# AUTOMATIC1111/stable-diffusion-webui

Hardware: AMD Instinct MI355X
Metric: images/sec SD1.5 512x512 20-step Euler-a, batch 8 per GPU (higher is better)
Workload: dtype f16

## Files before the change

### include/sdmi.h

```cpp
#ifndef SDMI_H
#define SDMI_H

#include <stdint.h>

#ifdef __cplusplus
extern "C" {
#endif

#define SDMI_VERSION 100

enum { SDMI_F16 = 0, SDMI_F32 = 1 };

typedef struct sdmi_engine sdmi_engine;

int sdmi_version(void);
const char* sdmi_last_error(void);
int sdmi_device_ok(void);


int64_t sdmi_attention_workspace_bytes(int B, int H, int M, int D);
int sdmi_attention(const void* q, const void* k, const void* v, void* out,
                   int B, int H, int N, int M, int D,
                   int ldq, int ldk, int ldv, int ldo, float scale,
                   void* workspace, int64_t workspace_bytes, void* stream);
// ... 32 lines not shown
    int32_t force_generic;
    int32_t reserved;
    void* splitk_workspace;
    int64_t splitk_workspace_bytes;
} sdmi_conv_desc;

enum {
    SDMI_EP_OUT_F32  = 1,
    SDMI_EP_GEGLU    = 2,
    SDMI_EP_NCHW     = 4,
    SDMI_EP_BIAS_ROW = 8,
    SDMI_EP_WRAP = 128,
    SDMI_EP_TRANSPOSE = 64
};
int sdmi_conv_gemm(const sdmi_conv_desc* d, void* stream);
int64_t sdmi_conv_splitk_workspace_bytes(int M, int N, int K, int batch);

int sdmi_pack_conv_weight(const void* w_oihw, int dtype, void* out_f16, int O, int I, int kh, int kw,
                          int O_pad, int I_pad, int geglu, void* stream);

int sdmi_groupnorm(const void* x0, const void* x1, int c0, int c1, const void* gamma_f32, const void* beta_f32,
                   void* out_f16, int B, int HW, int groups, float eps, int silu,
                   void* workspace_f32, int64_t workspace_bytes, void* stream);
int64_t sdmi_groupnorm_workspace_bytes(int B, int HW, int groups);

int sdmi_layernorm(const void* x, const void* gamma_f32, const void* beta_f32, void* out_f16,
                   int64_t rows, int C, float eps, void* stream);

int64_t sdmi_rowchain_ff_pack_bytes(int C, int hidden);
int sdmi_rowchain_ff_pack(const void* w1_f16, const void* b1_f32_or_null, const void* w2_f16, void* packs, int C, int hidden,
                          void* stream);
int sdmi_rowchain_ff(const void* x_f16, void* out_f16, const void* ln_gamma_f32, const void* ln_beta_f32, const void* packs,
                     const void* b2_f32_or_null, int64_t rows, int C, int hidden, float eps, void* stream);


int sdmi_philox_randn(void* out_f32, int64_t n, uint64_t seed, uint32_t offset, void* stream);

int sdmi_slerp(void* out_f32, const void* low_f32, const void* high_f32, float val, int C, int H, int W, void* scratch_f32,
               void* stream);


int sdmi_cfg_prepare_input(const void* x_f32, const void* c_in_f32, void* x_in, int out_dtype,
                           int B, int reps, int64_t chw, void* stream);

int sdmi_cfg_prepare_concat(const void* x_f32, const void* c_in_f32, const void* c_concat_f32, void* x_in, int out_dtype,
                            int B, int reps, int C, int Cc, int64_t hw, uint32_t zero_reps, void* stream);

int sdmi_cfg_combine(const void* x_f32, const void* eps_f32, const void* c_out_f32, float cond_scale, int mode,
                     const void* mask_f32, const void* nmask_f32, const void* init_latent_f32,
                     void* denoised_f32, int B, int64_t chw, void* stream);

int sdmi_cfg_combine_affine(const void* x_f32, const void* out_f32, const void* c_out_f32, const void* c_skip_f32,
                            float cond_scale, const void* mask_f32, const void* nmask_f32, const void* init_latent_f32,
                            void* denoised_f32, int B, int64_t chw, void* stream);

int sdmi_euler_step(void* x_f32, const void* denoised_f32, const void* noise_f32_or_null,
                    float sigma, float sigma_down, float sigma_up, float s_noise, int64_t n, void* stream);

int sdmi_dpmpp2m_step(void* x_f32, const void* denoised_f32, const void* old_denoised_f32_or_null,
                      float ratio, float em1, float c1, float c2, int64_t n, void* stream);

int sdmi_ddim_step(void* x_f32, const void* e_t_f32, const void* noise_f32_or_null, void* pred_x0_f32_or_null,
                   float a_t, float a_prev, float sigma_t, float sqrt_one_minus_at, int64_t n, void* stream);

int sdmi_axpby(void* y_f32, const void* x_f32, float a, const void* z_f32_or_null, float b, int64_t n, void* stream);

// ... 218 lines not shown
```

### stable-diffusion-webui_amd/_lib.py

```python
from __future__ import annotations

import ctypes as C
import os
import re

_HERE = os.path.dirname(os.path.abspath(__file__))
LIB_PATH = os.environ.get("SDMI_LIB") or os.path.join(_HERE, "lib", "libsdmi.so")
HEADER_PATH = os.path.join(os.path.dirname(_HERE), "include", "sdmi.h")

F16, F32 = 0, 1
EP_OUT_F32, EP_GEGLU, EP_NCHW, EP_BIAS_ROW = 1, 2, 4, 8
EP_TRANSPOSE = 64
EP_WRAP = 128
RRDB_EP_NONE, RRDB_EP_LRELU, RRDB_EP_RES1, RRDB_EP_RES2 = 0, 1, 2, 3
RRDB_ST_F16, RRDB_ST_F32_NCHW, RRDB_ST_U8_HWC = 0, 1, 2
COMPACT_EP_NONE, COMPACT_EP_PRELU, COMPACT_EP_TAIL = 0, 1, 2


class SdmiError(RuntimeError):
    pass


class ConvDesc(C.Structure):
    _fields_ = [
# ... 66 lines not shown
def declared_symbols() -> list:
    src = open(HEADER_PATH).read()
    src = re.sub(r"/\*.*?\*/", "", src, flags=re.S)
    return sorted(set(re.findall(r"\b(sdmi_[a-z0-9_]+)\s*\(", src)))


if not os.path.exists(LIB_PATH):
    raise ImportError(
        f"{LIB_PATH} is missing: build it with `python -c 'import __graft_entry__ as g; g.build()'` "
        "(hipcc --offload-arch=gfx950). There is no CPU fallback for the MI355X engine.")

lib = C.CDLL(LIB_PATH)

_vp, _i, _i64, _f, _u32 = C.c_void_p, C.c_int, C.c_int64, C.c_float, C.c_uint32
_SIGS = {
    "sdmi_version": (C.c_int, []),
    "sdmi_last_error": (C.c_char_p, []),
    "sdmi_device_ok": (C.c_int, []),
    "sdmi_attention_workspace_bytes": (_i64, [_i, _i, _i, _i]),
    "sdmi_attention": (_i, [_vp, _vp, _vp, _vp, _i, _i, _i, _i, _i, _i, _i, _i, _i, _f, _vp, _i64, _vp]),
    "sdmi_attention_wide_workspace_bytes": (_i64, [_i, _i, _i, _i]),
    "sdmi_attention_wide": (_i, [_vp, _vp, _vp, _vp, _i, _i, _i, _i, _i, _i, _i, _i, _f, _vp, _i64, _vp]),
    "sdmi_attention_vt": (_i, [_vp, _vp, _vp, _vp, _i, _i, _i, _i, _i, _i, _i, _i, _i, _f, _i, _vp]),
    "sdmi_conv_gemm": (_i, [C.POINTER(ConvDesc), _vp]),
    "sdmi_conv_splitk_workspace_bytes": (_i64, [_i, _i, _i, _i]),
    "sdmi_bench_conv_gemm": (_i, [C.POINTER(ConvDesc), _i, C.POINTER(C.c_float), _vp]),
    "sdmi_pack_conv_weight": (_i, [_vp, _i, _vp, _i, _i, _i, _i, _i, _i, _i, _vp]),
    "sdmi_groupnorm": (_i, [_vp, _vp, _i, _i, _vp, _vp, _vp, _i, _i, _i, _f, _i, _vp, _i64, _vp]),
    "sdmi_groupnorm_workspace_bytes": (_i64, [_i, _i, _i]),
    "sdmi_layernorm": (_i, [_vp, _vp, _vp, _vp, _i64, _i, _f, _vp]),
    "sdmi_rowchain_ff_pack_bytes": (_i64, [_i, _i]),
    "sdmi_rowchain_ff_pack": (_i, [_vp, _vp, _vp, _vp, _i, _i, _vp]),
    "sdmi_rowchain_ff": (_i, [_vp, _vp, _vp, _vp, _vp, _vp, _i64, _i, _i, _f, _vp]),
    "sdmi_philox_randn": (_i, [_vp, _i64, C.c_uint64, C.c_uint32, _vp]),
    "sdmi_slerp": (_i, [_vp, _vp, _vp, _f, _i, _i, _i, _vp, _vp]),
    "sdmi_cfg_prepare_input": (_i, [_vp, _vp, _vp, _i, _i, _i, _i64, _vp]),
    "sdmi_cfg_prepare_concat": (_i, [_vp, _vp, _vp, _vp, _i, _i, _i, _i, _i, _i64, _u32, _vp]),
    "sdmi_cfg_combine": (_i, [_vp, _vp, _vp, _f, _i, _vp, _vp, _vp, _vp, _i, _i64, _vp]),
    "sdmi_cfg_combine_affine": (_i, [_vp, _vp, _vp, _vp, _f, _vp, _vp, _vp, _vp, _i, _i64, _vp]),
    "sdmi_euler_step": (_i, [_vp, _vp, _vp, _f, _f, _f, _f, _i64, _vp]),
    "sdmi_dpmpp2m_step": (_i, [_vp, _vp, _vp, _f, _f, _f, _f, _i64, _vp]),
    "sdmi_ddim_step": (_i, [_vp, _vp, _vp, _vp, _f, _f, _f, _f, _i64, _vp]),
    "sdmi_axpby": (_i, [_vp, _vp, _f, _vp, _f, _i64, _vp]),
    "sdmi_dpm_error_partials": (_i, [_vp, _vp, _vp, _f, _f, _vp, _i64, _vp]),
    "sdmi_lincomb": (_i, [_vp, C.POINTER(_vp), C.POINTER(_f), _i, _i64, _vp]),
    "sdmi_mask_blend": (_i, [_vp, _vp, _vp, _vp, _i64, _vp]),
    "sdmi_latent_resize": (_i, [_vp, _vp, _i, _i, _i, _i, _i, _i, _vp]),
    "sdmi_image_to_u8": (_i, [_vp, _vp, _i, _i, _i, _i, _vp]),
    "sdmi_engine_create": (_vp, [_i]),
    "sdmi_engine_destroy": (None, [_vp]),
    "sdmi_unet_configure": (_i, [_vp, C.POINTER(UNetConfigC)]),
    "sdmi_unet_load_tensor": (_i, [_vp, C.c_char_p, _vp, _i, _i, C.POINTER(C.c_int64), _i]),
    "sdmi_unet_finalize": (_i, [_vp]),
    "sdmi_clip_configure": (_i, [_vp, _i, C.POINTER(ClipConfigC)]),
    "sdmi_clip_load_tensor": (_i, [_vp, _i, C.c_char_p, _vp, _i, _i, C.POINTER(C.c_int64), _i]),
    "sdmi_clip_finalize": (_i, [_vp, _i]),
    "sdmi_clip_forward": (_i, [_vp, _i, _vp, _vp, _i, _i, _i, _i, _vp, _vp, _vp]),
    "sdmi_unet_update_weight": (_i, [_vp, C.c_char_p, _vp, _i, _i, C.POINTER(C.c_int64), _i]),
    "sdmi_unet_hypernet_clear": (_i, [_vp]),
    "sdmi_unet_hypernet_begin": (_i, [_vp, _f]),
    "sdmi_unet_hypernet_linear": (_i, [_vp, _i, _i, _vp, _vp, _i, _i, _i, _i]),
    "sdmi_unet_hypernet_act": (_i, [_vp, _i, _i, _i]),
    "sdmi_unet_hypernet_layernorm": (_i, [_vp, _i, _i, _vp, _vp, _i, _i, _i]),
    "sdmi_unet_update_vector": (_i, [_vp, C.c_char_p, _vp, _i, _i64, _i]),
    "sdmi_lora_merge": (_i, [_vp, _vp, _i, _vp, _i, _vp, _i, _i, _i, _i, _f, _vp]),
    "sdmi_weight_hadamard": (_i, [_vp, _vp, _vp, _vp, _f, _i64, _vp]),
# ... 83 lines not shown
```

### stable-diffusion-webui_amd/csrc/capi.cpp

```cpp
#include "engine.h"
#include "prof.h"
#include <cstring>

namespace sdmi {
extern int g_vae_attn_rows;
int unet_forward(sdmi_engine* e, const void* x, const void* t, const void* ctx, const void* y, void* out, int io_dtype,
                 int Bn, int h, int w, int L, hipStream_t s);
int vae_decode(sdmi_engine* e, const void* z, int io_dtype, float* out, int B, int h, int w, hipStream_t s);
int vae_encode(sdmi_engine* e, const void* x, int io_dtype, float* out, int B, int H, int W, hipStream_t s);
int engine_load_unet_tensor(sdmi_engine* e, const char* key, const void* data, int dtype, int ndim, const int64_t* shape, int on_device);
int engine_load_vae_tensor(sdmi_engine* e, const char* key, const void* data, int dtype, int ndim, const int64_t* shape, int on_device);
int engine_unet_finalize(sdmi_engine* e);
int engine_clip_configure(sdmi_engine* e, int slot, const sdmi_clip_config* cfg);
int engine_clip_load_tensor(sdmi_engine* e, int slot, const char* key, const void* data, int dtype, int ndim, const int64_t* shape, int on_device);
int engine_clip_finalize(sdmi_engine* e, int slot);
int engine_clip_forward(sdmi_engine* e, int slot, const int* tokens, const float* inputs_embeds, int B, int L, int skip,
                        int apply_final_ln, float* out, float* pooled, hipStream_t s);
int engine_unet_update_weight(sdmi_engine* e, const char* key, const void* data, int dtype, int ndim, const int64_t* shape, int on_device);
int engine_vae_finalize(sdmi_engine* e);
int engine_hypernet_clear(sdmi_engine* e);
int engine_hypernet_begin(sdmi_engine* e, float multiplier);
int engine_hypernet_linear(sdmi_engine* e, int dim, int which, const void* w, const void* b, int dtype, int out_f, int in_f, int on_device);
int engine_hypernet_act(sdmi_engine* e, int dim, int which, int act);
int engine_hypernet_layernorm(sdmi_engine* e, int dim, int which, const void* g, const void* b, int dtype, int n, int on_device);
// ... 202 lines not shown

int64_t sdmi_groupnorm_workspace_bytes(int B, int HW, int groups) { return groupnorm_ws_bytes(B, HW, groups); }

int sdmi_groupnorm(const void* x0, const void* x1, int c0, int c1, const void* gamma, const void* beta, void* out, int B, int HW,
                   int groups, float eps, int silu, void* ws, int64_t ws_bytes, void* stream) {
    API_GUARD_BEGIN
    SDMI_REQUIRE(ws && ws_bytes >= groupnorm_ws_bytes(B, HW, groups), "groupnorm workspace too small");
    return launch_groupnorm((const half_t*)x0, (const half_t*)x1, c0, x1 ? c1 : 0, (const float*)gamma, (const float*)beta,
                            (half_t*)out, B, HW, groups, eps, silu != 0, (float*)ws, (hipStream_t)stream);
    API_GUARD_END
}

int sdmi_layernorm(const void* x, const void* gamma, const void* beta, void* out, int64_t rows, int C, float eps, void* stream) {
    API_GUARD_BEGIN
    return launch_layernorm((const half_t*)x, (const float*)gamma, (const float*)beta, (half_t*)out, rows, C, eps, (hipStream_t)stream);
    API_GUARD_END
}

int64_t sdmi_rowchain_ff_pack_bytes(int C, int hidden) { return (int64_t)rowchain_ff_pack_bytes(C, hidden); }
int sdmi_rowchain_ff_pack(const void* w1, const void* b1, const void* w2, void* packs, int C, int hidden, void* stream) {
    API_GUARD_BEGIN
    SDMI_REQUIRE(w1 && w2 && packs, "null argument");
    return launch_rowchain_ff_pack((const half_t*)w1, (const float*)b1, (const half_t*)w2, packs, C, hidden, false, (hipStream_t)stream);
    API_GUARD_END
}
int sdmi_rowchain_ff(const void* x, void* out, const void* g, const void* b, const void* packs, const void* b2, int64_t rows, int C,
                     int hidden, float eps, void* stream) {
    API_GUARD_BEGIN
    SDMI_REQUIRE(x && out && g && b && packs, "null argument");
    return launch_rowchain_ff((const half_t*)x, (half_t*)out, (const float*)g, (const float*)b, packs, (const float*)b2, (long)rows, C,
                              hidden, eps, (hipStream_t)stream);
    API_GUARD_END
}


int sdmi_philox_randn(void* out, int64_t n, uint64_t seed, uint32_t offset, void* stream) {
    API_GUARD_BEGIN
    return launch_philox((float*)out, n, seed, offset, (hipStream_t)stream);
    API_GUARD_END
}

int sdmi_slerp(void* out, const void* low, const void* high, float val, int C, int H, int W, void* scratch, void* stream) {
    API_GUARD_BEGIN
    SDMI_REQUIRE(out && low && high && scratch && C > 0 && H > 0 && W > 0, "bad arguments");
    return launch_slerp((float*)out, (const float*)low, (const float*)high, val, C, H, W, (float*)scratch, (hipStream_t)stream);
    API_GUARD_END
}

int sdmi_cfg_prepare_input(const void* x, const void* c_in, void* x_in, int out_dtype, int B, int reps, int64_t chw, void* stream) {
    API_GUARD_BEGIN
    return launch_cfg_prepare((const float*)x, (const float*)c_in, x_in, out_dtype, B, reps, chw, (hipStream_t)stream);
    API_GUARD_END
}

int sdmi_cfg_prepare_concat(const void* x, const void* c_in, const void* c_concat, void* x_in, int out_dtype, int B, int reps,
                            int C, int Cc, int64_t hw, uint32_t zero_reps, void* stream) {
    API_GUARD_BEGIN
    SDMI_REQUIRE(x && c_concat && x_in, "null pointer");
    SDMI_REQUIRE(B > 0 && reps > 0 && reps <= 32 && C > 0 && Cc > 0 && hw > 0, "bad sizes");
    return launch_cfg_prepare_concat((const float*)x, (const float*)c_in, (const float*)c_concat, x_in, out_dtype, B, reps, C, Cc, hw,
                                     zero_reps, (hipStream_t)stream);
    API_GUARD_END
}

int sdmi_cfg_combine(const void* x, const void* eps, const void* c_out, float cond_scale, int mode, const void* mask,
                     const void* nmask, const void* init_latent, void* den, int B, int64_t chw, void* stream) {
// ... 532 lines not shown
```

### stable-diffusion-webui_amd/csrc/common.h

```cpp
#pragma once
#include <hip/hip_runtime.h>
#include <stdint.h>
#include <string>

typedef _Float16 half_t;
typedef _Float16 h8 __attribute__((ext_vector_type(8)));
typedef _Float16 h4 __attribute__((ext_vector_type(4)));
typedef _Float16 h2 __attribute__((ext_vector_type(2)));
typedef float f4 __attribute__((ext_vector_type(4)));
typedef float f16v __attribute__((ext_vector_type(16)));

namespace sdmi {

#ifndef SDMI_GELU_SIG
#define SDMI_GELU_SIG 1
#endif
__device__ __forceinline__ float geglu_gate(float val, float g) {
    const float gc = fminf(fmaxf(g, -10.0f), 10.0f);
    const float g2 = gc * gc;
    float p = fmaf(1.01426306e-3f, g2, -0.106775724f);
    p = fmaf(p, g2, -2.30112135f);
    const float e = __builtin_amdgcn_exp2f(p * gc);
    return (val * g) * __builtin_amdgcn_rcpf(1.0f + e);
}
// ... 116 lines not shown
extern int g_gemm_pipe_default;
extern int g_force_gemm_split;
extern int g_attn_kvt;
extern int g_attn_occ;
extern int g_attn_lds_pad;
extern int g_attn_fold_min_m;
extern int g_attn_tau;
extern unsigned long long g_attn_dbg;
extern int g_gemm_dbgflags;
extern unsigned long long g_gemm_dbg;

struct AttnP {
    const half_t* q;
    const half_t* k;
    const half_t* vt;
    half_t* out;
    int B, H, N, M, D;
    int ldq, ldk, vt_ld, ldo;
    float scale_log2;
    int causal;
    long long* dbg;
    float tau;
};
int launch_attention(const AttnP& p, bool force_generic, hipStream_t s);
int launch_transpose_v(const half_t* v, half_t* vt, int B, int H, int M, int D, int ldv, int Mpad, hipStream_t s);

bool rowchain_supports(int C);
size_t rowchain_ff_pack_bytes(int C, int hidden);
int launch_rowchain_ff_pack(const half_t* w1, const float* b1, const half_t* w2, void* packs, int C, int hidden, bool permuted,
                            hipStream_t s);
int launch_rowchain_ff(const half_t* x, half_t* out, const float* gamma, const float* beta, const void* packs, const float* bias_out,
                       long rows, int C, int hidden, float eps, hipStream_t s);

enum { RRDB_EP_NONE = 0, RRDB_EP_LRELU = 1,
       RRDB_EP_RES1 = 2,
       RRDB_EP_RES2 = 3 };
enum { RRDB_ST_F16 = 0, RRDB_ST_F32_NCHW = 1, RRDB_ST_U8_HWC = 2 };
struct RrdbP {
    const half_t* in;
    const half_t* w;
    const float* bias;
    const half_t* r1;
    const half_t* r2;
    void* out;
    const half_t* zero;
    int B, H, W;
    int cin, lda, ldw, up;
    int ldo, n_real, ldr1, ldr2;
    int ep, store;
    float alpha, beta;
    long long M;
};
int launch_rrdb_conv(const RrdbP& p, int nout, hipStream_t s);
int launch_rrdb_input(const void* in, int u8, half_t* out, int B, int C, int H, int W, int f, int cpad, hipStream_t s);

enum { COMPACT_EP_NONE = 0, COMPACT_EP_PRELU = 1,
       COMPACT_EP_TAIL = 2 };
struct CompactP {
    const half_t* in;
    const half_t* w;
    const float* bias;
    const float* slope;
    const void* base;
    void* out;
    const half_t* zero;
    int B, H, W;
// ... 92 lines not shown
```

### stable-diffusion-webui_amd/csrc/engine.cpp

```cpp
#include "engine.h"

#include <algorithm>
#include <cmath>
#include <cstring>
#include <functional>

namespace sdmi {

static thread_local std::string g_err;
void set_error(const std::string& m) { g_err = m; }
const char* get_error() { return g_err.c_str(); }

const half_t* zero_page() {
    static thread_local int cached_dev = -1;
    static thread_local half_t* cached = nullptr;
    static std::map<int, half_t*> pages;
    int dev = 0;
    if (hipGetDevice(&dev) != hipSuccess) return nullptr;
    if (dev == cached_dev) return cached;
    auto it = pages.find(dev);
    if (it == pages.end()) {
        void* p = nullptr;
        if (hipMalloc(&p, kZeroPageHalfs * sizeof(half_t)) != hipSuccess) return nullptr;
        if (hipMemset(p, 0, kZeroPageHalfs * sizeof(half_t)) != hipSuccess) return nullptr;
// ... 661 lines not shown
            TRY(run_linear(r, b.qk1, n1, (int)M1, nullptr, qk, 2 * C));
            half_t* vt = r.H((size_t)B * C * Npad);
            TRY(run_vt(r, b.v1, n1, C, B1, HW, Npad, vt, false));
            a1 = r.H(M * C);
            TRY(run_attn(r, qk, qk + C, vt, a1, B1, st.heads, HW, HW, st.dhead, 2 * C, 2 * C, Npad, C));
        } else {
            auto alloc = [&](size_t n) { return r.H(n); };
            const half_t *xk = nullptr, *xv = nullptr;
            TRY(run_hn(r, C, 0, n1, M, alloc, false, &xk));
            TRY(run_hn(r, C, 1, n1, M, alloc, false, &xv));
            ConvW wq = b.qk1, wk = b.qk1;
            wq.n_pad = wk.n_pad = C; wq.cout = wk.cout = C;
            wk.w = b.qk1.w + (size_t)C * b.qk1.cin_pad;
            if (b.qk1.b) wk.b = b.qk1.b + C;
            half_t* q = r.H(M * C);
            half_t* k = r.H(M * C);
            TRY(run_linear(r, wq, n1, (int)M, nullptr, q, C));
            TRY(run_linear(r, wk, xk, (int)M, nullptr, k, C));
            half_t* vt = r.H((size_t)B * C * Npad);
            TRY(run_vt(r, b.v1, xv, C, B, HW, Npad, vt, false));
            a1 = r.H(M * C);
            TRY(run_attn(r, q, k, vt, a1, B, st.heads, HW, HW, st.dhead, C, C, Npad, C));
        }
        half_t* x1 = r.S(M * C);
        r.lnp_want = fold && e->ln_fold >= 2;
        TRY(run_linear(r, b.o1, a1, (int)M1, cur, x1, C, 1.f, false, r.lo(cur, MC), r.lo(x1, MC)));
        if (B1 != B) {
            if (!r.dry) SDMI_CHECK_HIP(hipMemcpyAsync(x1 + M1 * C, x1, M1 * C * sizeof(half_t), hipMemcpyDeviceToDevice, r.s));
            if (!r.dry && acc) SDMI_CHECK_HIP(hipMemcpyAsync(x1 + MC + M1 * C, x1 + MC, M1 * C * sizeof(half_t), hipMemcpyDeviceToDevice, r.s));
            B1 = B; M1 = M;
        }
        r.tap(bname + ".attn1+x", x1, B, H, Wd, C);
        const bool chain_ok = !fold && !acc && !e->force_generic && e->use_glds && rowchain_supports(C) && HW % 128 == 0 && e->n_streams <= 1;
        half_t* x2 = nullptr;
        {
        half_t* q2 = nullptr;
        if (fold) {
            LnStats st2;
            TRY(run_ln_stats(r, b.ln2, x1, M, &st2));
            q2 = r.H(M * C);
            TRY(run_linear_ln(r, b.q2, b.ln2, x1, st2, (int)M, q2, C));
        } else {
            half_t* n2 = r.H(M * C);
            TRY(run_ln(r, b.ln2, x1, M, n2, r.lo(x1, MC)));
            q2 = r.H(M * C);
            TRY(run_linear(r, b.q2, n2, (int)M, nullptr, q2, C));
        }
        half_t* a2 = r.H(M * C);
        if (!r.dry) {
            SDMI_REQUIRE(e->ctx_valid && e->ctx_B == (r.Btot ? r.Btot : B), "context not set for this batch size");
            AttnP p{};
            p.q = q2; p.out = a2;
            p.k = e->ctx_k[b.ctx_slot] + (size_t)r.b0 * e->ctx_L * C;
            p.vt = e->ctx_vt[b.ctx_slot] + (size_t)r.b0 * C * e->ctx_Lpad;
            p.B = B; p.H = st.heads; p.N = HW; p.M = e->ctx_L; p.D = st.dhead;
            p.ldq = C; p.ldk = C; p.vt_ld = e->ctx_Lpad; p.ldo = C;
            p.scale_log2 = (1.0f / sqrtf((float)st.dhead)) * 1.4426950408889634f;
            TRY(launch_attention(p, e->force_generic, r.s));
        }
        x2 = r.S(M * C);
        r.lnp_want = fold && e->ln_fold >= 2;
        TRY(run_linear(r, b.o2, a2, (int)M, x1, x2, C, 1.f, false, r.lo(x1, MC), r.lo(x2, MC)));
        }
        r.tap(bname + ".attn2+x", x2, B, H, Wd, C);
        half_t* x3 = reuse ? pp[blk & 1] : r.S(M * C);
        if (chain_ok && (e->fuse_rows & 2) && b.ff1.geglu && b.ff1.n_pad % 64 == 0 && b.ff2.cin_pad * 2 == b.ff1.n_pad && b.ff1.cin_pad == C &&
            b.ff2.n_pad == C) {
            if (!r.dry) {
// ... 1523 lines not shown
}

sdmi_compact::~sdmi_compact() {
    for (void* p : owned) (void)hipFree(p);
}

sdmi_esrgan::~sdmi_esrgan() {
    for (void* p : owned) (void)hipFree(p);
}

sdmi_engine::~sdmi_engine() {
    (void)hipSetDevice(device);
    (void)hipDeviceSynchronize();
    sdmi::free_raw(raw_unet);
    sdmi::free_raw(raw_vae);
    sdmi::free_raw(raw_clip[0]);
    sdmi::free_raw(raw_clip[1]);
    sdmi::ctx_free(this);
    for (void* p : owned) (void)hipFree(p);
    for (void* p : owned_vae) (void)hipFree(p);
    for (void* p : owned_hn) (void)hipFree(p);
    if (hn_ctx_scratch) (void)hipFree(hn_ctx_scratch);
    if (arena.base) (void)hipFree(arena.base);
    for (auto& a : aux_arenas) if (a.base) (void)hipFree(a.base);
    for (hipStream_t st : aux_streams) (void)hipStreamDestroy(st);
    for (hipEvent_t ev : ev_join) (void)hipEventDestroy(ev);
    if (ev_fork) (void)hipEventDestroy(ev_fork);
}

#ifndef __HIP__
#include "rrdb.hip"
#include "compact.hip"
#include "swinir.hip"
#endif
```

### stable-diffusion-webui_amd/csrc/engine.h

```cpp
#pragma once
#include "common.h"
#include "../../include/sdmi.h"

#include <cstdlib>
#include <map>
#include <memory>
#include <string>
#include <vector>

namespace sdmi {

struct RawTensor {
    void* ptr = nullptr;
    int dtype = 0;
    std::vector<int64_t> shape;
    size_t bytes = 0;
};

struct ConvW {
    half_t* w = nullptr;
    float* b = nullptr;
    int cin = 0, cin_pad = 0, cout = 0, n_pad = 0, taps = 1;
    bool geglu = false;
    mutable half_t* w_ln = nullptr;
// ... 126 lines not shown

}

struct sdmi_engine {
    int device = 0;
    std::map<std::string, sdmi::RawTensor> raw_unet, raw_vae;
    struct PackSite { half_t* dst; int O, cin, kh, Opad, cin_pad, geglu; };
    std::map<std::string, std::vector<PackSite>> unet_sites;
    struct VecSite { float* dst; int n, n_pad, geglu; };
    std::map<std::string, std::vector<VecSite>> unet_vec_sites;
    bool recording_unet_sites = false;
    std::vector<void*> owned;
    std::vector<void*> owned_vae;
    std::vector<void*>* alloc_sink = nullptr;
    std::vector<sdmi::HnNet> hypernets;
    std::vector<void*> owned_hn;
    char* hn_ctx_scratch = nullptr;
    size_t hn_ctx_scratch_bytes = 0;
    sdmi::UNetW unet;
    sdmi::VAEW vae;
    sdmi::ClipW clip[2];
    std::map<std::string, sdmi::RawTensor> raw_clip[2];
    sdmi::Arena arena;
    int n_streams = 1;
    int arena_reuse = 0;
    std::vector<hipStream_t> aux_streams;
    std::vector<sdmi::Arena> aux_arenas;
    std::vector<hipEvent_t> ev_join;
    hipEvent_t ev_fork = nullptr;
    bool force_generic = false;
    bool use_glds = true;
    float vae_stream_scale = 1.f;
    int ln_fold = 0;
    int fuse_rows = [] { const char* e = getenv("SDMI_FUSE_ROWS"); return e ? atoi(e) : 2; }();
    bool residual_fp32 = false;
    long weights_epoch = 0;
    bool cfg_pairs = false;
    bool uniform_t = false;
    bool auto_promises = false;
    bool tiling = false;
    bool trace = false;
    struct Tap { std::string name; const half_t* ptr; int B, H, W, C; };
    std::vector<Tap> taps;
    std::vector<const void*> control;
    std::vector<int64_t> control_numel;
    bool only_mid_control = false;
    half_t* ctx_f16 = nullptr;
    std::vector<half_t*> ctx_k;
    std::vector<half_t*> ctx_vt;
    std::vector<void*> ctx_owned;
    int ctx_B = 0, ctx_L = 0, ctx_Lpad = 0;
    bool ctx_valid = false;
    int* ctx_gate = nullptr;

    ~sdmi_engine();
};

struct sdmi_esrgan {
    struct Conv { half_t* w = nullptr; float* b = nullptr; int cin = 0, nout = 0, n_real = 0; };
    sdmi_engine* e = nullptr;
    int num_block = 0, in_ch = 0, scale = 0;
    int unshuffle = 1;
    int cin0 = 0;
    Conv first, body, up1, up2, hr, last;
    std::vector<Conv> rdb;
    std::vector<void*> owned;
    ~sdmi_esrgan();
// ... 31 lines not shown
```

### stable-diffusion-webui_amd/ops.py

```python
from __future__ import annotations

import ctypes as C
from typing import Optional

import torch

from . import _lib
from ._lib import lib, check, ptr, stream_ptr, ConvDesc, F16, F32, EP_OUT_F32, EP_GEGLU, EP_NCHW, EP_BIAS_ROW


def _rup(x, m):
    return (x + m - 1) // m * m


def attention(q: torch.Tensor, k: torch.Tensor, v: torch.Tensor, heads: int, scale: Optional[float] = None) -> torch.Tensor:
    _lib.require_device()
    assert q.dtype == torch.float16 and k.dtype == torch.float16 and v.dtype == torch.float16
    b, n, c = q.shape
    m = k.shape[1]
    d = c // heads
    q, k, v = [t if t.stride(-1) == 1 and t.stride(0) == t.shape[1] * t.stride(1) else t.contiguous() for t in (q, k, v)]
    out = torch.empty((b, n, c), dtype=torch.float16, device=q.device)
    scale = d ** -0.5 if scale is None else scale
    if heads == 1 and d > 160 and d % 64 == 0:
# ... 125 lines not shown

def layernorm(x: torch.Tensor, gamma: torch.Tensor, beta: torch.Tensor, eps: float = 1e-5) -> torch.Tensor:
    _lib.require_device()
    c = x.shape[-1]
    x = x.contiguous()
    out = torch.empty_like(x)
    check(lib.sdmi_layernorm(ptr(x), ptr(gamma.float().contiguous()), ptr(beta.float().contiguous()), ptr(out),
                             x.numel() // c, c, float(eps), stream_ptr()), "sdmi_layernorm")
    return out


def rowchain_ff_pack(w1: torch.Tensor, b1, w2: torch.Tensor) -> torch.Tensor:
    _lib.require_device()
    hidden, c = w2.shape[1], w2.shape[0]
    w1, w2 = w1.half().contiguous(), w2.half().contiguous()
    b1 = b1.float().contiguous() if b1 is not None else None
    packs = torch.empty(int(lib.sdmi_rowchain_ff_pack_bytes(c, hidden)), dtype=torch.uint8, device=w1.device)
    check(lib.sdmi_rowchain_ff_pack(ptr(w1), ptr(b1) if b1 is not None else None, ptr(w2), ptr(packs), c, hidden, stream_ptr()),
          "sdmi_rowchain_ff_pack")
    return packs


def rowchain_ff(x: torch.Tensor, gamma, beta, packs: torch.Tensor, b2, hidden: int, eps: float = 1e-5) -> torch.Tensor:
    _lib.require_device()
    c = x.shape[-1]
    x = x.contiguous()
    out = torch.empty_like(x)
    b2 = b2.float().contiguous() if b2 is not None else None
    check(lib.sdmi_rowchain_ff(ptr(x), ptr(out), ptr(gamma.float().contiguous()), ptr(beta.float().contiguous()), ptr(packs),
                               ptr(b2) if b2 is not None else None, x.numel() // c, c, hidden, float(eps), stream_ptr()), "sdmi_rowchain_ff")
    return out


def philox_randn(shape, seed: int, offset: int, device) -> torch.Tensor:
    _lib.require_device()
    out = torch.empty(tuple(shape), dtype=torch.float32, device=device)
    check(lib.sdmi_philox_randn(ptr(out), out.numel(), C.c_uint64(seed & 0xFFFFFFFFFFFFFFFF), C.c_uint32(offset), stream_ptr()),
          "sdmi_philox_randn")
    return out


def lincomb(out: torch.Tensor, terms, coefs) -> torch.Tensor:
    _lib.require_device()
    n = len(terms)
    assert 1 <= n <= 6 and len(coefs) == n
    for t in terms:
        assert t.dtype == torch.float32 and t.is_contiguous() and t.numel() == out.numel()
    assert out.dtype == torch.float32 and out.is_contiguous()
    tarr = (C.c_void_p * n)(*[t.data_ptr() for t in terms])
    carr = (C.c_float * n)(*[float(c) for c in coefs])
    check(lib.sdmi_lincomb(ptr(out), tarr, carr, n, out.numel(), stream_ptr()), "sdmi_lincomb")
    return out


def mask_blend(x: torch.Tensor, init: torch.Tensor, mask: torch.Tensor, nmask: torch.Tensor) -> torch.Tensor:
    _lib.require_device()
    m = mask.to(x.device, torch.float32).expand_as(x).contiguous()
    nm = nmask.to(x.device, torch.float32).expand_as(x).contiguous()
    init = init.to(x.device, torch.float32).expand_as(x).contiguous()
    check(lib.sdmi_mask_blend(ptr(x), ptr(init), ptr(m), ptr(nm), x.numel(), stream_ptr()), "sdmi_mask_blend")
    return x


def latent_resize(x: torch.Tensor, size, mode: str = "bilinear", antialias: bool = False) -> torch.Tensor:
    _lib.require_device()
    x = x.float().contiguous()
# ... 154 lines not shown
```

Before: 21.69.

## Fuse cross-attention LayerNorm, Q projection, attention and output projection into one kernel

Adds a single HIP kernel that, per 128-row tile, applies LayerNorm, multiplies by Wq, runs flash-style cross-attention against the precomputed context K and V^T, then applies Wo plus bias and the residual. Weight and key/value tiles stream into shared memory through a three-stage ring. It is enabled by default (fuse_rows now 3) for the C=320, 8-head, d=40 transformer blocks. This removes the global-memory round trips and extra launches between the separate LN, GEMM, attention and GEMM kernels. The cost is a specialized, register-heavy kernel with low occupancy that only covers the highest-resolution cross-attention blocks.

```diff
diff --git a/include/sdmi.h b/include/sdmi.h
--- a/include/sdmi.h
+++ b/include/sdmi.h
@@ -88,6 +88,10 @@
                           void* stream);
 int sdmi_rowchain_ff(const void* x_f16, void* out_f16, const void* ln_gamma_f32, const void* ln_beta_f32, const void* packs,
                      const void* b2_f32_or_null, int64_t rows, int C, int hidden, float eps, void* stream);
+
+int sdmi_xattn_chain(const void* x_f16, void* out_f16, const void* ln_gamma_f32, const void* ln_beta_f32, const void* wq_f16,
+                     const void* wo_f16, const void* bo_f32_or_null, const void* k_f16, const void* vt_f16, int64_t rows,
+                     int rows_per_image, int C, int heads, int L, int Lpad, float eps, void* stream);
 
 
 int sdmi_philox_randn(void* out_f32, int64_t n, uint64_t seed, uint32_t offset, void* stream);
diff --git a/stable-diffusion-webui_amd/_lib.py b/stable-diffusion-webui_amd/_lib.py
--- a/stable-diffusion-webui_amd/_lib.py
+++ b/stable-diffusion-webui_amd/_lib.py
@@ -122,6 +122,7 @@
     "sdmi_rowchain_ff_pack_bytes": (_i64, [_i, _i]),
     "sdmi_rowchain_ff_pack": (_i, [_vp, _vp, _vp, _vp, _i, _i, _vp]),
     "sdmi_rowchain_ff": (_i, [_vp, _vp, _vp, _vp, _vp, _vp, _i64, _i, _i, _f, _vp]),
+    "sdmi_xattn_chain": (_i, [_vp, _vp, _vp, _vp, _vp, _vp, _vp, _vp, _vp, _i64, _i, _i, _i, _i, _i, _f, _vp]),
     "sdmi_philox_randn": (_i, [_vp, _i64, C.c_uint64, C.c_uint32, _vp]),
     "sdmi_slerp": (_i, [_vp, _vp, _vp, _f, _i, _i, _i, _vp, _vp]),
     "sdmi_cfg_prepare_input": (_i, [_vp, _vp, _vp, _i, _i, _i, _i64, _vp]),
diff --git a/stable-diffusion-webui_amd/csrc/capi.cpp b/stable-diffusion-webui_amd/csrc/capi.cpp
--- a/stable-diffusion-webui_amd/csrc/capi.cpp
+++ b/stable-diffusion-webui_amd/csrc/capi.cpp
@@ -258,6 +258,14 @@
                               hidden, eps, (hipStream_t)stream);
     API_GUARD_END
 }
+int sdmi_xattn_chain(const void* x, void* out, const void* g, const void* b, const void* wq, const void* wo, const void* bo, const void* k,
+                     const void* vt, int64_t rows, int rows_per_image, int C, int heads, int L, int Lpad, float eps, void* stream) {
+    API_GUARD_BEGIN
+    return launch_xattn_chain((const half_t*)x, (half_t*)out, (const float*)g, (const float*)b, (const half_t*)wq, (const half_t*)wo,
+                              (const float*)bo, (const half_t*)k, (const half_t*)vt, (long)rows, rows_per_image, C, heads, L, Lpad, eps,
+                              (hipStream_t)stream);
+    API_GUARD_END
+}
 
 
 int sdmi_philox_randn(void* out, int64_t n, uint64_t seed, uint32_t offset, void* stream) {
diff --git a/stable-diffusion-webui_amd/csrc/common.h b/stable-diffusion-webui_amd/csrc/common.h
--- a/stable-diffusion-webui_amd/csrc/common.h
+++ b/stable-diffusion-webui_amd/csrc/common.h
@@ -172,6 +172,10 @@
 int launch_rowchain_ff(const half_t* x, half_t* out, const float* gamma, const float* beta, const void* packs, const float* bias_out,
                        long rows, int C, int hidden, float eps, hipStream_t s);
 
+int launch_xattn_chain(const half_t* x, half_t* out, const float* gamma, const float* beta, const half_t* wq, const half_t* wo,
+                       const float* bo, const half_t* k, const half_t* vt, long rows, int rows_per_image, int C, int heads, int L, int Lpad,
+                       float eps, hipStream_t s);
+
 enum { RRDB_EP_NONE = 0, RRDB_EP_LRELU = 1,
        RRDB_EP_RES1 = 2,
        RRDB_EP_RES2 = 3 };
diff --git a/stable-diffusion-webui_amd/csrc/engine.cpp b/stable-diffusion-webui_amd/csrc/engine.cpp
--- a/stable-diffusion-webui_amd/csrc/engine.cpp
+++ b/stable-diffusion-webui_amd/csrc/engine.cpp
@@ -717,8 +717,18 @@
         }
         r.tap(bname + ".attn1+x", x1, B, H, Wd, C);
         const bool chain_ok = !fold && !acc && !e->force_generic && e->use_glds && rowchain_supports(C) && HW % 128 == 0 && e->n_streams <= 1;
+        const bool xchain = chain_ok && (e->fuse_rows & 1) && !hn_has_dim(e, C) && st.heads == 8 && st.dhead == 40 && !b.q2.b &&
+                            b.q2.cin_pad == C && b.q2.n_pad == C && b.o2.cin_pad == C && b.o2.n_pad == C;
         half_t* x2 = nullptr;
-        {
+        if (xchain) {
+            x2 = r.S(M * C);
+            if (!r.dry) {
+                SDMI_REQUIRE(e->ctx_valid && e->ctx_B == (r.Btot ? r.Btot : B), "context not set for this batch size");
+                TRY(launch_xattn_chain(x1, x2, b.ln2.g, b.ln2.b, b.q2.w, b.o2.w, b.o2.b, e->ctx_k[b.ctx_slot] + (size_t)r.b0 * e->ctx_L * C,
+                                       e->ctx_vt[b.ctx_slot] + (size_t)r.b0 * C * e->ctx_Lpad, (long)M, HW, C, st.heads, e->ctx_L,
+                                       e->ctx_Lpad, 1e-5f, r.s));
+            }
+        } else {
         half_t* q2 = nullptr;
         if (fold) {
             LnStats st2;
@@ -2308,4 +2318,5 @@
 #include "rrdb.hip"
 #include "compact.hip"
 #include "swinir.hip"
+#include "xattn_chain.hip"
 #endif
diff --git a/stable-diffusion-webui_amd/csrc/engine.h b/stable-diffusion-webui_amd/csrc/engine.h
--- a/stable-diffusion-webui_amd/csrc/engine.h
+++ b/stable-diffusion-webui_amd/csrc/engine.h
@@ -182,7 +182,7 @@
     bool use_glds = true;
     float vae_stream_scale = 1.f;
     int ln_fold = 0;
-    int fuse_rows = [] { const char* e = getenv("SDMI_FUSE_ROWS"); return e ? atoi(e) : 2; }();
+    int fuse_rows = [] { const char* e = getenv("SDMI_FUSE_ROWS"); return e ? atoi(e) : 3; }();
     bool residual_fp32 = false;
     long weights_epoch = 0;
     bool cfg_pairs = false;
diff --git a/stable-diffusion-webui_amd/csrc/xattn_chain.hip b/stable-diffusion-webui_amd/csrc/xattn_chain.hip
--- /dev/null
+++ b/stable-diffusion-webui_amd/csrc/xattn_chain.hip
@@ -0,0 +1,383 @@
+#include "common.h"
+#include "prof.h"
+
+#include <algorithm>
+#include <cmath>
+
+namespace sdmi {
+
+#ifdef __HIP__
+typedef const __attribute__((address_space(1))) void* xgptr_t;
+typedef __attribute__((address_space(3))) void* xlptr_t;
+#define XC_WAIT_VM3() asm volatile("s_waitcnt vmcnt(3) lgkmcnt(0)" ::: "memory")
+#define XC_WAIT_VM0() asm volatile("s_waitcnt vmcnt(0) lgkmcnt(0)" ::: "memory")
+#define XC_FENCE() asm volatile("" ::: "memory")
+#define XC_REAL_BRANCH() asm volatile("")
+#define XC_OPAQUE(x) asm volatile("" : "+v"(x))
+#else
+typedef const void* xgptr_t;
+typedef void* xlptr_t;
+#define XC_WAIT_VM3() ((void)0)
+#define XC_WAIT_VM0() ((void)0)
+#define XC_FENCE() ((void)0)
+#define XC_REAL_BRANCH() ((void)0)
+#define XC_OPAQUE(x) ((void)0)
+#endif
+
+constexpr int kXcC = 320, kXcD = 40, kXcRows = 128;
+constexpr int kXcRowBytes = kXcC * 2;
+constexpr int kXcImage = kXcRows * kXcRowBytes;
+constexpr int kXcStage = 24 * 1024;
+constexpr int kXcLds = kXcImage + 3 * kXcStage;
+
+struct XattnP {
+    const half_t* x;
+    half_t* out;
+    const float* gamma;
+    const float* beta;
+    const half_t* wq;
+    const half_t* wo;
+    const float* bo;
+    const half_t* k;
+    const half_t* vt;
+    int rows_per_image;
+    int L, Lpad;
+    float eps, scale_log2, tau;
+};
+
+__device__ __forceinline__ int xc_img(int row, int col) { return row * kXcRowBytes + ((((col >> 3) ^ ((row >> 1) & 7))) << 4) + (col & 7) * 2; }
+
+__global__ __launch_bounds__(512) void rowchain_xattn_kernel(const XattnP p) {
+#ifdef __HIP__
+    extern __shared__ __attribute__((aligned(16))) char smem[];
+#else
+    __shared__ __attribute__((aligned(16))) char smem[kXcLds];
+#endif
+    char* const img = smem;
+    char* const ring = smem + kXcImage;
+    const int tid = threadIdx.x, lane = tid & 63;
+    const int wave = __builtin_amdgcn_readfirstlane(tid >> 6);
+    const int wr = wave >> 2, wc = wave & 3;
+    const int l16 = lane & 15, q4 = lane >> 4;
+    const int lq = lane & 31, half = lane >> 5;
+    const long row0 = (long)blockIdx.x * kXcRows;
+    const int image = (int)(row0 / p.rows_per_image);
+    const half_t* const kimg = p.k + (long)image * p.L * kXcC;
+    const half_t* const vimg = p.vt + (long)image * kXcC * p.Lpad;
+    const int nblk = (p.L + 31) >> 5;
+    const int nsteps = 20 + 2 * nblk;
+
+    auto stage_cols = [&](const half_t* w, int ld, int k0, char* buf) {
+        int ln = lane;
+        XC_OPAQUE(ln);
+#pragma unroll
+        for (int u = 0; u < 3; ++u) {
+            const int pb = u * 8 + wave;
+            const int n = pb * 16 + (ln >> 2);
+            const int seg = (ln & 3) ^ (3 * ((n >> 3) & 1));
+            const half_t* src = w + (long)min(n, kXcC - 1) * ld + k0 + seg * 8;
+            __builtin_amdgcn_global_load_lds((xgptr_t)src, (xlptr_t)(buf + pb * 1024), 16, 0, 0);
+        }
+    };
+    auto stage_keys = [&](int key0, char* buf) {
+        int ln = lane;
+        XC_OPAQUE(ln);
+#pragma unroll
+        for (int u = 0; u < 3; ++u) {
+            const int pb = u * 8 + wave;
+            const int pc = pb * 64 + ln;
+            const int r = pc / 40, ps = pc - r * 40;
+            const int rr = min(r, 31);
+            const int key = min(key0 + rr, p.L - 1);
+            const half_t* src = kimg + (long)key * kXcC + ((ps ^ ((rr >> 1) & 7)) << 3);
+            __builtin_amdgcn_global_load_lds((xgptr_t)src, (xlptr_t)(buf + pb * 1024), 16, 0, 0);
+        }
+    };
+    auto issue = [&](int seq) {
+        if (seq >= nsteps) return;
+        char* buf = ring + (seq % 3) * kXcStage;
+        if (seq < 10) stage_cols(p.wq, kXcC, seq * 32, buf);
+        else if (seq < 10 + 2 * nblk) {
+            const int blk = (seq - 10) >> 1;
+            if ((seq - 10) & 1) stage_cols(vimg, p.Lpad, blk * 32, buf);
+            else stage_keys(blk * 32, buf);
+        } else stage_cols(p.wo, kXcC, (seq - 10 - 2 * nblk) * 32, buf);
+    };
+    auto open_step = [&](int s) -> const char* {
+        if (s + 1 < nsteps) XC_WAIT_VM3(); else XC_WAIT_VM0();
+        __builtin_amdgcn_s_barrier();
+        XC_FENCE();
+        issue(s + 2);
+        return ring + (s % 3) * kXcStage;
+    };
+
+    issue(0);
+    issue(1);
+
+    {
+        const int sub = tid & 7;
+        const float inv_c = 1.0f / (float)kXcC;
+        h8 v[2][5];
+#pragma unroll
+        for (int ps = 0; ps < 2; ++ps) {
+            const half_t* src = p.x + (row0 + ps * 64 + (tid >> 3)) * kXcC + sub * 8;
+#pragma unroll
+            for (int i = 0; i < 5; ++i) v[ps][i] = *reinterpret_cast<const h8*>(src + i * 64);
+        }
+#pragma unroll
+        for (int ps = 0; ps < 2; ++ps) {
+            const int row = ps * 64 + (tid >> 3);
+            float a = 0.f;
+#pragma unroll
+            for (int i = 0; i < 5; ++i)
+#pragma unroll
+                for (int e = 0; e < 8; ++e) a += (float)v[ps][i][e];
+            for (int off = 4; off > 0; off >>= 1) a += __shfl_xor(a, off);
+            const float mean = a * inv_c;
+            float sq = 0.f;
+#pragma unroll
+            for (int i = 0; i < 5; ++i)
+#pragma unroll
+                for (int e = 0; e < 8; ++e) { const float d = (float)v[ps][i][e] - mean; sq = fmaf(d, d, sq); }
+            for (int off = 4; off > 0; off >>= 1) sq += __shfl_xor(sq, off);
+            const float rstd = rsqrtf(fmaf(sq, inv_c, p.eps));
+#pragma unroll
+            for (int i = 0; i < 5; ++i) {
+                const int c0 = (i * 8 + sub) * 8;
+                const f4 g0 = *reinterpret_cast<const f4*>(p.gamma + c0), g1 = *reinterpret_cast<const f4*>(p.gamma + c0 + 4);
+                const f4 b0 = *reinterpret_cast<const f4*>(p.beta + c0), b1 = *reinterpret_cast<const f4*>(p.beta + c0 + 4);
+                h8 o;
+#pragma unroll
+                for (int e = 0; e < 8; ++e) {
+                    const float g = e < 4 ? g0[e] : g1[e - 4], bb = e < 4 ? b0[e] : b1[e - 4];
+                    o[e] = (half_t)(((float)v[ps][i][e] - mean) * rstd * g + bb);
+                }
+                *reinterpret_cast<h8*>(img + xc_img(row, c0)) = o;
+            }
+        }
+    }
+
+    const int a_off = (64 * wr + l16) * kXcRowBytes, a_sw = (l16 >> 1) & 7;
+    const int w_off = (80 * wc + l16) * 64 + ((q4 ^ (3 * (l16 >> 3))) << 4);
+    f4 acc[4][5];
+    auto zero_acc = [&]() {
+#pragma unroll
+        for (int mi = 0; mi < 4; ++mi)
+#pragma unroll
+            for (int j = 0; j < 5; ++j) acc[mi][j] = f4{0.f, 0.f, 0.f, 0.f};
+    };
+    auto gemm_step = [&](const char* buf, int kc) {
+        h8 af[4], wf[5];
+#pragma unroll
+        for (int j = 0; j < 5; ++j) wf[j] = *reinterpret_cast<const h8*>(buf + w_off + j * 1024);
+#pragma unroll
+        for (int mi = 0; mi < 4; ++mi) af[mi] = *reinterpret_cast<const h8*>(img + a_off + mi * 16 * kXcRowBytes + (((kc * 4 + q4) ^ a_sw) << 4));
+#pragma unroll
+        for (int mi = 0; mi < 4; ++mi)
+#pragma unroll
+            for (int j = 0; j < 5; ++j) acc[mi][j] = __builtin_amdgcn_mfma_f32_16x16x32_f16(wf[j], af[mi], acc[mi][j], 0, 0, 0);
+    };
+
+    zero_acc();
+    int s = 0;
+#pragma unroll 1
+    for (; s < 10; ++s) {
+        const char* buf = open_step(s);
+        gemm_step(buf, s);
+    }
+
+    const char* kb = open_step(s++);
+#pragma unroll
+    for (int mi = 0; mi < 4; ++mi)
+#pragma unroll
+        for (int j = 0; j < 5; ++j) {
+            const h4 hv = {(half_t)acc[mi][j][0], (half_t)acc[mi][j][1], (half_t)acc[mi][j][2], (half_t)acc[mi][j][3]};
+            *reinterpret_cast<h4*>(img + xc_img(64 * wr + 16 * mi + l16, 80 * wc + 16 * j + 4 * q4)) = hv;
+        }
+    XC_FENCE();
+    __builtin_amdgcn_wave_barrier();
+    f16v o[4][2];
+    float m_run[4];
+    h8 pb[4][2];
+#pragma unroll
+    for (int st = 0; st < 4; ++st) {
+        m_run[st] = -1e30f;
+#pragma unroll
+        for (int db = 0; db < 2; ++db)
+#pragma unroll
+            for (int r = 0; r < 16; ++r) o[st][db][r] = 0.f;
+    }
+    const int krow = (lq & 0x13) | ((lq & 4) << 1) | ((lq & 8) >> 1);
+    const int k_off = krow * kXcRowBytes, k_sw = (krow >> 1) & 7, q_sw = (lq >> 1) & 7;
+    const h8 ones = {(half_t)1.f, (half_t)1.f, (half_t)1.f, (half_t)1.f, (half_t)1.f, (half_t)1.f, (half_t)1.f, (half_t)1.f};
+    const h8 zeros = {0, 0, 0, 0, 0, 0, 0, 0};
+#pragma unroll 1
+    for (int blk = 0; blk < nblk; ++blk) {
+        if (blk > 0) kb = open_step(s++);
+        const bool ragged = blk * 32 + 32 > p.L;
+        const int lim = p.L - blk * 32 - 8 * half;
+#pragma unroll
+        for (int st = 0; st < 4; ++st) {
+            const int hs = (2 * wc + (st >> 1)) * 5;
+            const int qrow = 64 * wr + 32 * (st & 1) + lq;
+            f16v sc;
+#pragma unroll
+            for (int r = 0; r < 16; ++r) sc[r] = 0.f;
+#pragma unroll
+            for (int dc = 0; dc < 3; ++dc) {
+                const bool padk = dc == 2 && half == 1;
+                const int c = hs + dc * 2 + (dc == 2 ? 0 : half);
+                h8 qf = *reinterpret_cast<const h8*>(img + qrow * kXcRowBytes + ((c ^ q_sw) << 4));
+                if (padk) qf = zeros;
+                const h8 kf = *reinterpret_cast<const h8*>(kb + k_off + ((c ^ k_sw) << 4));
+                sc = __builtin_amdgcn_mfma_f32_32x32x16_f16(kf, qf, sc, 0, 0, 0);
+            }
+            if (ragged) {
+                XC_REAL_BRANCH();
+#pragma unroll
+                for (int r = 0; r < 16; ++r)
+                    if (16 * (r >> 3) + (r & 7) >= lim) sc[r] = -INFINITY;
+            }
+            float mx = -INFINITY;
+#pragma unroll
+            for (int r = 0; r < 16; ++r) mx = fmaxf(mx, sc[r]);
+            float mlo = mx, mhi = mx;
+#ifdef __HIP__
+            asm volatile("s_nop 1\n\tv_permlane32_swap_b32 %0, %1" : "+v"(mlo), "+v"(mhi));
+#else
+            emu_permlane32_swap(mlo, mhi);
+#endif
+            mx = fmaxf(mlo, mhi) * p.scale_log2;
+            const bool moved = p.tau < 0.f || __builtin_amdgcn_ballot_w64(mx > m_run[st] + fmaxf(p.tau, 0.f)) != 0;
+            const float m_new = moved ? fmaxf(m_run[st], mx) : m_run[st];
+            const float alpha = __builtin_amdgcn_exp2f(m_run[st] - m_new);
+            m_run[st] = m_new;
+#pragma unroll
+            for (int r = 0; r < 16; ++r) pb[st][r >> 3][r & 7] = (half_t)__builtin_amdgcn_exp2f(fmaf(sc[r], p.scale_log2, -m_new));
+            if (moved) {
+#pragma unroll
+                for (int db = 0; db < 2; ++db)
+#pragma unroll
+                    for (int r = 0; r < 16; ++r) o[st][db][r] *= alpha;
+            }
+            __builtin_amdgcn_sched_barrier(0);
+        }
+        const char* vb = open_step(s++);
+#pragma unroll
+        for (int h2 = 0; h2 < 2; ++h2) {
+            h8 vf[2][2];
+#pragma unroll
+            for (int db = 0; db < 2; ++db)
+#pragma unroll
+                for (int sb = 0; sb < 2; ++sb) {
+                    const int n = (2 * wc + h2) * kXcD + db * 32 + lq;
+                    vf[db][sb] = *reinterpret_cast<const h8*>(vb + n * 64 + (((sb * 2 + half) ^ (3 * ((n >> 3) & 1))) << 4));
+                    if (db == 1 && lq == 8) vf[db][sb] = ones;
+                }
+#pragma unroll
+            for (int qb = 0; qb < 2; ++qb)
+#pragma unroll
+                for (int db = 0; db < 2; ++db)
+#pragma unroll
+                    for (int sb = 0; sb < 2; ++sb)
+                        o[h2 * 2 + qb][db] = __builtin_amdgcn_mfma_f32_32x32x16_f16(vf[db][sb], pb[h2 * 2 + qb][sb], o[h2 * 2 + qb][db], 0, 0, 0);
+            __builtin_amdgcn_sched_barrier(0);
+        }
+    }
+#pragma unroll
+    for (int st = 0; st < 4; ++st) {
+        const float l_tot = __shfl(o[st][1][4], lq);
+        const float inv = 1.0f / l_tot;
+        const int qrow = 64 * wr + 32 * (st & 1) + lq;
+        const int col0 = (2 * wc + (st >> 1)) * kXcD;
+#pragma unroll
+        for (int db = 0; db < 2; ++db)
+#pragma unroll
+            for (int g = 0; g < 4; ++g) {
+                if (db * 32 + g * 8 >= kXcD) continue;
+                h4 hv;
+#pragma unroll
+                for (int e = 0; e < 4; ++e) hv[e] = (half_t)(o[st][db][g * 4 + e] * inv);
+                *reinterpret_cast<h4*>(img + xc_img(qrow, col0 + db * 32 + g * 8 + half * 4)) = hv;
+            }
+    }
+
+    zero_acc();
+#pragma unroll 1
+    for (int kc = 0; kc < 10; ++kc) {
+        const char* buf = open_step(s++);
+        gemm_step(buf, kc);
+    }
+    XC_WAIT_VM0();
+    __builtin_amdgcn_s_barrier();
+    XC_FENCE();
+#pragma unroll
+    for (int u = 0; u < 10; ++u) {
+        const int pc = u * 512 + tid;
+        const int r = pc / 40, ps = pc - r * 40;
+        const half_t* src = p.x + (row0 + r) * kXcC + ((ps ^ ((r >> 1) & 7)) << 3);
+        __builtin_amdgcn_global_load_lds((xgptr_t)src, (xlptr_t)(img + (u * 8 + wave) * 1024), 16, 0, 0);
+    }
+    XC_WAIT_VM0();
+    __builtin_amdgcn_s_barrier();
+    XC_FENCE();
+#pragma unroll
+    for (int j = 0; j < 5; ++j) {
+        const int col = 80 * wc + 16 * j + 4 * q4;
+        const f4 bb = *reinterpret_cast<const f4*>(p.bo + col);
+#pragma unroll
+        for (int mi = 0; mi < 4; ++mi) {
+            h4* cell = reinterpret_cast<h4*>(img + xc_img(64 * wr + 16 * mi + l16, col));
+            const h4 res = *cell;
+            h4 hv;
+#pragma unroll
+            for (int e = 0; e < 4; ++e) hv[e] = (half_t)((acc[mi][j][e] + bb[e]) + (float)res[e]);
+            *cell = hv;
+        }
+    }
+    XC_WAIT_VM0();
+    __builtin_amdgcn_s_barrier();
+    XC_FENCE();
+#pragma unroll
+    for (int u = 0; u < 10; ++u) {
+        const int pc = u * 512 + tid;
+        const int r = pc / 40, ps = pc - r * 40;
+        const h8 hv = *reinterpret_cast<const h8*>(img + pc * 16);
+        *reinterpret_cast<h8*>(p.out + (row0 + r) * kXcC + ((ps ^ ((r >> 1) & 7)) << 3)) = hv;
+    }
+}
+
+int launch_xattn_chain(const half_t* x, half_t* out, const float* gamma, const float* beta, const half_t* wq, const half_t* wo,
+                       const float* bo, const half_t* k, const half_t* vt, long rows, int rows_per_image, int C, int heads, int L, int Lpad,
+                       float eps, hipStream_t s) {
+    SDMI_REQUIRE(C == kXcC, "cross-attention chain: built for row width C = 320");
+    SDMI_REQUIRE(heads * kXcD == C, "cross-attention chain: heads * 40 == C (8 heads of 40)");
+    SDMI_REQUIRE(rows > 0 && rows % kXcRows == 0, "cross-attention chain: rows % 128 == 0");
+    SDMI_REQUIRE(rows_per_image > 0 && rows_per_image % kXcRows == 0 && rows % rows_per_image == 0,
+                 "cross-attention chain: rows_per_image % 128 == 0 (a tile lies in one image) and whole images");
+    SDMI_REQUIRE(x && out && gamma && beta && wq && wo && k && vt, "cross-attention chain: null pointer");
+    SDMI_REQUIRE(L >= 1, "cross-attention chain: context length L >= 1");
+    SDMI_REQUIRE(Lpad >= L && Lpad % 32 == 0, "cross-attention chain: Lpad >= L, a multiple of 32 (whole 32-key blocks of V^T)");
+    SDMI_REQUIRE(rows / kXcRows < (1l << 31), "cross-attention chain: too many tiles");
+    SDMI_REQUIRE((((uintptr_t)x | (uintptr_t)out | (uintptr_t)gamma | (uintptr_t)beta | (uintptr_t)wq | (uintptr_t)wo | (uintptr_t)bo |
+                   (uintptr_t)k | (uintptr_t)vt) & 15) == 0, "cross-attention chain: 16-byte aligned operands");
+    XattnP p{};
+    p.x = x; p.out = out; p.gamma = gamma; p.beta = beta; p.wq = wq; p.wo = wo;
+    p.bo = bo ? bo : reinterpret_cast<const float*>(zero_page());
+    p.k = k; p.vt = vt; p.rows_per_image = rows_per_image; p.L = L; p.Lpad = Lpad; p.eps = eps;
+    p.scale_log2 = (1.0f / sqrtf((float)kXcD)) * 1.4426950408889634f;
+    p.tau = (float)(g_attn_tau < 0 ? -1 : g_attn_tau > 12 ? 12 : g_attn_tau);
+    ProfScope ps("rowchain_xattn", 4.0 * (double)rows * C * C, 4.0 * (double)rows * C + 4.0 * C * C, s);
+    auto kern = rowchain_xattn_kernel;
+#ifdef __HIP__
+    static PerDeviceOnce attr;
+    if (attr.need()) SDMI_CHECK_HIP(hipFuncSetAttribute((const void*)kern, hipFuncAttributeMaxDynamicSharedMemorySize, kXcLds));
+    hipLaunchKernelGGL(kern, dim3((unsigned)(rows / kXcRows)), dim3(512), kXcLds, s, p);
+#else
+    hipLaunchKernelGGL(kern, dim3((unsigned)(rows / kXcRows)), dim3(512), 0, s, p);
+#endif
+    SDMI_CHECK_HIP(hipGetLastError());
+    return 0;
+}
+
+}
diff --git a/stable-diffusion-webui_amd/ops.py b/stable-diffusion-webui_amd/ops.py
--- a/stable-diffusion-webui_amd/ops.py
+++ b/stable-diffusion-webui_amd/ops.py
@@ -181,6 +181,20 @@
     return out
 
 
+def xattn_chain(x: torch.Tensor, gamma, beta, wq: torch.Tensor, wo: torch.Tensor, bo, k: torch.Tensor, vt: torch.Tensor, L: int,
+                heads: int = 8, eps: float = 1e-5) -> torch.Tensor:
+    _lib.require_device()
+    images, rpi, c = x.shape
+    x = x.contiguous()
+    out = torch.empty_like(x)
+    wq, wo, k, vt = wq.half().contiguous(), wo.half().contiguous(), k.half().contiguous(), vt.half().contiguous()
+    bo = bo.float().contiguous() if bo is not None else None
+    check(lib.sdmi_xattn_chain(ptr(x), ptr(out), ptr(gamma.float().contiguous()), ptr(beta.float().contiguous()), ptr(wq), ptr(wo),
+                               ptr(bo) if bo is not None else None, ptr(k), ptr(vt), images * rpi, rpi, c, heads, int(L), vt.shape[-1],
+                               float(eps), stream_ptr()), "sdmi_xattn_chain")
+    return out
+
+
 def philox_randn(shape, seed: int, offset: int, device) -> torch.Tensor:
     _lib.require_device()
     out = torch.empty(tuple(shape), dtype=torch.float32, device=device)
```

After: 21.98 (median of 6 runs). +1.3%, better.
